# Blosc/c-blosc

Measured on NVIDIA H100. Metric: compress+decompress GB/s, higher is better.
Workload: dtype u8

## Files before the change

c-blosc_b200/csrc/dev_lz4.cuh:

```cuda
#pragma once
#include "dev_common.cuh"

#define LZ4_MFLIMIT 12
#define LZ4_LASTLITERALS 5
#define LZ4_TABLE_BYTES 16384
#define LZ4_TAB17_BYTES (8192 + 512)
#define LZ4_TAB17_MINLEN 65547
#define LZ4_TAB17_MAXLEN 131072

template <bool U16>
DEV u32 lz4_hash_at(const u8* __restrict__ s, int pos) {
  if (U16) return (ld_u32(s + pos) * 2654435761u) >> (32 - 13);
  const u64 seq = (u64)ld_u32(s + pos) | ((u64)s[pos + 4] << 32);
  return (u32)(((seq << 24) * 889523592379ull) >> (64 - 12));
}

#define LZ4_SCALAR_PROBES 4

DEV long long lz4_probe_offset(int it, int accel) {
  if (it == 0) return 0;
  const long long m = it - 1;
  const long long c = m >> 6;
  return 1 + m * accel + 32 * c * (c - 1) + c * (m - 64 * c);
}

struct StreamBase {
  const u8* s;
  const u32* s32;
  int sal;
  const uint4* s128;
  int sal16;
};
DEV StreamBase make_stream_base(const u8* s) {
  StreamBase b;
  b.s = s;
  b.s32 = (const u32*)((uintptr_t)s & ~(uintptr_t)3);
  b.sal = (int)((uintptr_t)s & 3u);
  b.s128 = (const uint4*)((uintptr_t)s & ~(uintptr_t)15);
  b.sal16 = (int)((uintptr_t)s & 15u);
  return b;
}
DEV void ldp_win12(const StreamBase& sb, int p, u32& b0, u32& b1, u32& b2) {
#ifdef SIMT_EMU
  memcpy(&b0, sb.s + p, 4); memcpy(&b1, sb.s + p + 4, 4); memcpy(&b2, sb.s + p + 8, 4);
#else
  const int q = p + sb.sal;
  const u32* w = sb.s32 + (q >> 2);
  const u32 sh = (u32)(q & 3) * 8u;
  const u32 w0 = __ldg(w), w1 = __ldg(w + 1), w2 = __ldg(w + 2), w3 = __ldg(w + 3);
  b0 = __funnelshift_r(w0, w1, sh); b1 = __funnelshift_r(w1, w2, sh); b2 = __funnelshift_r(w2, w3, sh);
#endif
}
DEV void ldp_raw12(const StreamBase& sb, int p, u32& r0, u32& r1, u32& r2, u32& r3) {
#ifdef SIMT_EMU
  memcpy(&r0, sb.s + p, 4); memcpy(&r1, sb.s + p + 4, 4); memcpy(&r2, sb.s + p + 8, 4); r3 = 0;
#else
  const u32* w = sb.s32 + ((p + sb.sal) >> 2);
  r0 = __ldg(w); r1 = __ldg(w + 1); r2 = __ldg(w + 2); r3 = __ldg(w + 3);
#endif
}
DEV void ldp_take12(const StreamBase& sb, int p, u32 r0, u32 r1, u32 r2, u32 r3, u32& b0, u32& b1, u32& b2) {
#ifdef SIMT_EMU
  (void)sb; (void)p; (void)r3; b0 = r0; b1 = r1; b2 = r2;
#else
  const u32 sh = (u32)((p + sb.sal) & 3) * 8u;
  b0 = __funnelshift_r(r0, r1, sh); b1 = __funnelshift_r(r1, r2, sh); b2 = __funnelshift_r(r2, r3, sh);
#endif
}
DEV void ldp_win8(const StreamBase& sb, int p, u32& b0, u32& b1) {
#ifdef SIMT_EMU
  memcpy(&b0, sb.s + p, 4); memcpy(&b1, sb.s + p + 4, 4);
#else
  const int q = p + sb.sal;
  const u32* w = sb.s32 + (q >> 2);
  const u32 sh = (u32)(q & 3) * 8u;
  const u32 w0 = __ldg(w), w1 = __ldg(w + 1), w2 = __ldg(w + 2);
  b0 = __funnelshift_r(w0, w1, sh); b1 = __funnelshift_r(w1, w2, sh);
#endif
}

DEV void ldp_raw20(const StreamBase& sb, int p, u32 (&r)[5]) {
#ifdef SIMT_EMU
  memcpy(&r[0], sb.s + p, 16); r[4] = sb.s[p + 16];
#else
  const u32* w = sb.s32 + ((p + sb.sal) >> 2);
  r[0] = __ldg(w); r[1] = __ldg(w + 1); r[2] = __ldg(w + 2); r[3] = __ldg(w + 3); r[4] = __ldg(w + 4);
#endif
}
DEV void ldp_take17(const StreamBase& sb, int p, const u32 (&r)[5], u32& a0, u32& a1, u32& a2, u32& a3, u32& a4b) {
#ifdef SIMT_EMU
  (void)sb; (void)p; a0 = r[0]; a1 = r[1]; a2 = r[2]; a3 = r[3]; a4b = r[4] & 0xffu;
#else
  const u32 sh = (u32)((p + sb.sal) & 3) * 8u;
  a0 = __funnelshift_r(r[0], r[1], sh); a1 = __funnelshift_r(r[1], r[2], sh);
  a2 = __funnelshift_r(r[2], r[3], sh); a3 = __funnelshift_r(r[3], r[4], sh);
  a4b = (r[4] >> sh) & 0xffu;
#endif
}
DEV void ldp_gather17(const StreamBase& sb, int p, u32& c0, u32& c1, u32& c2, u32& c3, u32& c4b) {
#ifdef SIMT_EMU
  memcpy(&c0, sb.s + p, 4); memcpy(&c1, sb.s + p + 4, 4); memcpy(&c2, sb.s + p + 8, 4); memcpy(&c3, sb.s + p + 12, 4);
  c4b = sb.s[p + 16];
#else
  const int q = p + sb.sal16;
  const uint4* w = sb.s128 + (q >> 4);
  const uint4 v0 = __ldg(w), v1 = __ldg(w + 1);
  const bool k1 = (q & 4) != 0, k2 = (q & 8) != 0;
  const u32 sh = (u32)(q & 3) * 8u;
  const u32 t0 = k1 ? v0.y : v0.x, t1 = k1 ? v0.z : v0.y, t2 = k1 ? v0.w : v0.z, t3 = k1 ? v1.x : v0.w;
  const u32 t4 = k1 ? v1.y : v1.x, t5 = k1 ? v1.z : v1.y, t6 = k1 ? v1.w : v1.z;
  const u32 u0 = k2 ? t2 : t0, u1 = k2 ? t3 : t1, u2 = k2 ? t4 : t2, u3 = k2 ? t5 : t3, u4 = k2 ? t6 : t4;
  c0 = __funnelshift_r(u0, u1, sh); c1 = __funnelshift_r(u1, u2, sh);
  c2 = __funnelshift_r(u2, u3, sh); c3 = __funnelshift_r(u3, u4, sh);
  c4b = (u4 >> sh) & 0xffu;
#endif
}

DEV void lz4d_prefetch(const u8* base, int p, int end) {
#ifndef SIMT_EMU
  if (p < end) asm volatile("prefetch.global.L1 [%0];" :: "l"(base + p));
#else
  (void)base; (void)p; (void)end;
#endif
}

DEV u32 ldp_win4(const StreamBase& sb, int p) {
#ifdef SIMT_EMU
  u32 b0; memcpy(&b0, sb.s + p, 4); return b0;
#else
  const int q = p + sb.sal;
  const u32* w = sb.s32 + (q >> 2);
  return __funnelshift_r(__ldg(w), __ldg(w + 1), (u32)(q & 3) * 8u);
#endif
}

template <bool U16>
DEV u32 lz4_hash_seq(u32 lo, u32 b4) {
  if (U16) return (lo * 2654435761u) >> (32 - 13);
  const u64 seq = (u64)lo | ((u64)(b4 & 0xffu) << 32);
  return (u32)(((seq << 24) * 889523592379ull) >> (64 - 12));
}

DEV int lz4_count_tail(const StreamBase& sb, const u8* __restrict__ s, int p, int q, int limit, int n) {
  if (p + 136 <= n) {
    const int lane = lane_id();
    const u32 x = ldp_win4(sb, p + 4 * lane) ^ ldp_win4(sb, q + 4 * lane);
    const unsigned full = __ballot_sync(FULLMASK, x == 0u);
    if (full != FULLMASK) {
      const int fl = __ffs((int)~full) - 1;
      return fl * 4 + eq_bytes32(__shfl_sync(FULLMASK, x, fl));
    }
    return 128 + warp_count_match(s, p + 128, q + 128, limit);
  }
  return warp_count_match(s, p, q, limit);
}

#ifdef SIMT_EMU
static long long g_dbg_lz4t_sessions = 0, g_dbg_lz4t_seqs = 0, g_dbg_lz4t_stale = 0, g_dbg_lz4t_x[6];
#define LZ4T_DBG(x) do { if (lane_id() == 0) (x)++; } while (0)
#else
#define LZ4T_DBG(x) do {} while (0)
#endif
#ifndef LZ4T_TILES
#define LZ4T_TILES 12
#endif
#ifndef LZ4T_AHEAD
#define LZ4T_AHEAD 8
#endif
#ifndef LZ4T_NAP
#define LZ4T_NAP 128
#endif
#define LZ4T_RING (32 * LZ4T_TILES)
#define LZ4T_BAR_IDLE(i) (1 + (i))
#define LZ4T_BAR_GO(i) (4 + (i))
#define LZ4T_QUIT 1
#define LZ4T_STOP 0x7fffffff
#define LZ4T_END 0xffffffffu
#define LZ4T_LONG 13
static_assert(LZ4T_TILES % 3 == 0 && LZ4T_AHEAD >= 1 && LZ4T_AHEAD < LZ4T_TILES && LZ4T_RING > 15 + 255 + 4, "team ring layout");
#define LZ4T_PREFETCH 512

enum {
  LZ4C_TOTAL,
  LZ4C_START,
  LZ4C_SESSION,
  LZ4C_FULLWAIT,
  LZ4C_REPROBE,
  LZ4C_SEARCH,
  LZ4C_SESSIONS, LZ4C_SEQS, LZ4C_CHAIN_SEQS,
  LZ4C_PREP_BUSY,
  LZ4C_PREP_OWN,
  LZ4C_PREP_GATHER,
  LZ4C_PREP_TILES,
  LZ4C_SMID, LZ4C_SUBP,
  LZ4C_STALE,
  LZ4C_N = 16
};
#ifdef B2_LZ4_CYCLES
#define LZ4C_MAXSTREAMS 16384
__device__ unsigned long long g_lz4_cycles[LZ4C_MAXSTREAMS][LZ4C_N];
#define LZ4C_T(t) const long long t = clock64()
#define LZ4C_TW(t) const long long t = TEAM ? clock64() : 0ll
#define LZ4C_ADD(k, v) do { if (lane_id() == 0) atomicAdd(&tm->cyc[k], (unsigned long long)(v)); } while (0)
#define LZ4C_SPAN(k, t) LZ4C_ADD(k, clock64() - (t))
#else
#define LZ4C_T(t) do {} while (0)
#define LZ4C_TW(t) do {} while (0)
#define LZ4C_ADD(k, v) do {} while (0)
#define LZ4C_SPAN(k, t) do {} while (0)
#endif

struct Lz4Team {
  uint2 vd[LZ4T_RING];
  int rdy[LZ4T_TILES];
  const u8* s;
  int n;
  int u16;
  int wt;
  int gen;
  int cmd;
  int sub[4];
  int slot;
#ifdef B2_LZ4_CYCLES
  unsigned long long cyc[LZ4C_N];
#endif
};
#define LZ4T_SMEM_BYTES ((int)sizeof(Lz4Team))

DEV int lz4t_ld_i32(const int* p) { return *(const volatile int*)p; }
DEV void lz4t_st_i32(int* p, int v) { *(volatile int*)p = v; }

template <bool U16>
DEV void lz4_team_prepare_tile(Lz4Team* tm, const void* tabmem, const u8* s, int n, int tile) {
  const int lane = lane_id();
  const int w0 = 32 * tile, p = w0 + lane;
  const int e = (tile % LZ4T_TILES) * 32 + lane;
  if (w0 + 31 + 24 > n) { tm->vd[e] = make_uint2(0u, LZ4T_END); return; }
  const StreamBase sb = make_stream_base(s);
  u32 r[5], a0, a1, a2, a3, a4, c0, c1, c2, c3, c4;
  LZ4C_T(c_t0);
  ldp_raw20(sb, p, r);
  ldp_take17(sb, p, r, a0, a1, a2, a3, a4);
  const u32 h = lz4_hash_seq<U16>(a0, a1);
  const int snap = U16 ? (int)((const volatile u16*)tabmem)[h] : (int)((const volatile u32*)tabmem)[h];
  u32 vx = h << 8, sn = LZ4T_END;
  if ((unsigned)snap < (unsigned)p) {
    LZ4C_T(c_t1);
    LZ4C_ADD(LZ4C_PREP_OWN, c_t1 - c_t0);
    ldp_gather17(sb, snap, c0, c1, c2, c3, c4);
    const u32 x1 = a1 ^ c1, x2 = a2 ^ c2, x3 = a3 ^ c3;
    u32 m;
    if (x1) m = (u32)(__ffs((int)x1) - 1) >> 3;
    else if (x2) m = 4u + ((u32)(__ffs((int)x2) - 1) >> 3);
    else if (x3) m = 8u + ((u32)(__ffs((int)x3) - 1) >> 3);
    else m = a4 != c4 ? 12u : (u32)LZ4T_LONG;
    const bool hit = (U16 || snap + 65535 >= p) && c0 == a0;
    vx |= (hit ? 1u : 0u) | (m << 2);
    sn = (u32)snap;
    LZ4C_SPAN(LZ4C_PREP_GATHER, c_t1);
  }
  tm->vd[e] = make_uint2(vx, sn);
}

DEV void lz4_team_preparer(Lz4Team* tm, const void* tabmem, int i) {
  for (;;) {
    bar_sync(LZ4T_BAR_GO(i), 64);
    if (lz4t_ld_i32(&tm->cmd) == LZ4T_QUIT) return;
    const u8* s = *(const u8* const volatile*)&tm->s;
    const int n = lz4t_ld_i32(&tm->n), u16 = lz4t_ld_i32(&tm->u16);
    for (int tile = i;; tile += 3) {
      int w;
      for (;;) {
        w = __shfl_sync(FULLMASK, lz4t_ld_i32(&tm->wt), 0);
        if (w == LZ4T_STOP) break;
        if (tile < w) tile = w + (i + 3 - w % 3) % 3;
        if (tile <= w + LZ4T_AHEAD) break;
        __nanosleep(LZ4T_NAP);
      }
      if (w == LZ4T_STOP) break;
      LZ4C_T(c_go);
      lz4d_prefetch(s, 32 * tile + LZ4T_PREFETCH + lane_id(), n);
      if (u16) lz4_team_prepare_tile<true>(tm, tabmem, s, n, tile);
      else lz4_team_prepare_tile<false>(tm, tabmem, s, n, tile);
      __syncwarp();
      if (lane_id() == 0) { __threadfence_block(); lz4t_st_i32(&tm->rdy[tile % LZ4T_TILES], tile + 1); }
      LZ4C_SPAN(LZ4C_PREP_BUSY, c_go);
      LZ4C_ADD(LZ4C_PREP_TILES, 1);
    }
    __syncwarp();
    bar_arrive(LZ4T_BAR_IDLE(i), 64);
  }
}

DEV void lz4t_reach(Lz4Team* tm, int ip, int& wt, int& vt) {
  const int lo = (ip - 2) >> 5, hi = ip >> 5;
  if (lo > wt + LZ4T_AHEAD) LZ4T_DBG(g_dbg_lz4t_x[2]);
  if (lo != wt) { wt = lo; lz4t_st_i32(&tm->wt, lo); }
  for (int t = vt + 1 > lo ? vt + 1 : lo; t <= hi; t++) {
    const int* r = &tm->rdy[t % LZ4T_TILES];
    if (lz4t_ld_i32(r) != t + 1) {
      LZ4T_DBG(g_dbg_lz4t_x[5]);
      do { __syncwarp(); } while (__any_sync(FULLMASK, lz4t_ld_i32(r) != t + 1));
    }
  }
  if (hi > vt) vt = hi;
}

template <bool U16, bool PACK, bool TEAM>
DEV int lz4_encode_stream(const u8* __restrict__ s, const int n, u8* __restrict__ d, const int cap,
                          const int accel, void* tabmem, int* need_out, Lz4Team* tm) {
  const int lane = lane_id();
  const StreamBase sb = make_stream_base(s);
  u16* tab16 = (u16*)tabmem;
  u32* tab32 = (u32*)tabmem;
  u32* tabhi = (u32*)((u8*)tabmem + 8192);
#define LZ4_TGET(h) (U16 ? (int)tab16[h] : PACK ? ((int)tab16[h] | (int)(((tabhi[(h) >> 5] >> ((h) & 31u)) & 1u) << 16)) : (int)tab32[h])
#define LZ4_TPUT(h, v) do { if (U16) tab16[h] = (u16)(v); else if (PACK) { tab16[h] = (u16)(v); const u32 m_ = 1u << ((h) & 31u); \
                            if ((v) & 0x10000) atomicOr(&tabhi[(h) >> 5], m_); else atomicAnd(&tabhi[(h) >> 5], ~m_); } \
                            else tab32[h] = (u32)(v); } while (0)

  for (int i = lane; i < (PACK ? LZ4_TAB17_BYTES : LZ4_TABLE_BYTES) / 4; i += 32) tab32[i] = 0;
  __syncwarp();

  const bool limited = (long long)cap < (long long)n + n / 255 + 16;
  const int olimit = cap;
  const int mfl1 = n - LZ4_MFLIMIT + 1;
  const int matchlimit = n - LZ4_LASTLITERALS;
  int ip = 1, anchor = 0, op = 0;
  int need = 0;
#define LZ4_LIMIT(v) do { const int v_ = (v); if (v_ > need) need = v_; if (limited && v_ > olimit) return 0; } while (0)

  int w0 = -(1 << 30);
  u32 wq0 = 0, wq1 = 0, wq2 = 0, wh = 0;
  int pb = -(1 << 30);
  u32 pq0 = 0, pq1 = 0, pq2 = 0, pq3 = 0;
  int nrec = 0, recop = 0;
  u32 rec = 0;
  int twt = 0, tvt = -1;
#define LZ4_FLUSH_CHECKED() do { if (nrec) { LZ4_LIMIT(op + (1 + LZ4_LASTLITERALS)); } LZ4_FLUSH(); } while (0)
#define LZ4_FLUSH() do { if (lane < nrec) { d[recop] = (u8)rec; d[recop + 1] = (u8)(rec >> 8); d[recop + 2] = (u8)(rec >> 16); \
                                             if ((rec & 15u) == 15u) d[recop + 3] = (u8)(rec >> 24); } nrec = 0; } while (0)

  if (n >= LZ4_MFLIMIT + 1) {
    bool post = false;
    for (;;) {
      int match = 0, lit = 0, back = 0;
      u32 ipn = 0, cn = 0;
      bool have_next = false, hit = false, imm = false, have_mc = false;
      int mc_carry = 0;

      bool scalar_post = post;
      if (TEAM && post && ip + 64 <= n) {
        scalar_post = false;
        bool finished = false;
        if (nrec >= 24) LZ4_FLUSH_CHECKED();
        LZ4T_DBG(g_dbg_lz4t_sessions);
        LZ4C_T(c_s0);
        LZ4C_ADD(LZ4C_SESSIONS, 1);
        if ((ip - 2) >> 5 <= twt + LZ4T_AHEAD) LZ4T_DBG(g_dbg_lz4t_x[3]);
        lz4t_reach(tm, ip, twt, tvt);
        __syncwarp();
        LZ4C_SPAN(LZ4C_START, c_s0);
        LZ4C_T(c_s1);
        const smem_addr_t vda = smem_addr(tm->vd);
        u32 e = (u32)ip % (u32)LZ4T_RING;
        for (;;) {
          u32 pk, snap;
          smem_ld_u32x2(vda, e << 3, pk, snap);
          const u32 h2 = smem_ld_u32(vda, (e >= 2u ? e - 2u : e - 2u + LZ4T_RING) << 3) >> 8;
          const u32 h = pk >> 8;
          LZ4_TPUT(h2, ip - 2);
          const int cand = LZ4_TGET(h);
          __syncwarp();
          if (cand != (int)snap) {
            LZ4T_DBG(g_dbg_lz4t_stale); LZ4C_ADD(LZ4C_STALE, 1);
            scalar_post = true; break;
          }
          LZ4_TPUT(h, ip);
          if (!(pk & 1u)) { LZ4T_DBG(g_dbg_lz4t_x[4]); ip++; break; }
          const int off = ip - (int)snap;
          int mc = (int)((pk >> 2) & 15u);
          if (mc == LZ4T_LONG) {
            LZ4T_DBG(g_dbg_lz4t_x[0]);
            mc = LZ4T_LONG + lz4_count_tail(sb, s, ip + 4 + LZ4T_LONG, ip - off + 4 + LZ4T_LONG, matchlimit, n);
            if (mc >= 15 + 255) {
              hit = true; imm = true; match = ip - off;
              have_mc = true; mc_carry = mc;
              LZ4T_DBG(g_dbg_lz4t_x[1]);
              break;
            }
          }
          const bool ext = mc >= 15;
          LZ4T_DBG(g_dbg_lz4t_seqs);
          LZ4C_ADD(LZ4C_CHAIN_SEQS, 1);
          if (lane == nrec) { rec = (ext ? 15u | ((u32)(mc - 15) << 24) : (u32)mc) | ((u32)off << 8); recop = op; }
          nrec++;
          op += ext ? 4 : 3;
          ip += mc + 4;
          e += (u32)(mc + 4);
          if (e >= (u32)LZ4T_RING) e -= (u32)LZ4T_RING;
          anchor = ip;
          if (ip + 64 > n) {
            if (ip >= mfl1) finished = true;
            else scalar_post = true;
            break;
          }
          if ((ip >> 5) > tvt) {
            LZ4C_T(c_w);
            lz4t_reach(tm, ip, twt, tvt);
            LZ4C_SPAN(LZ4C_FULLWAIT, c_w);
            if (nrec >= 24) LZ4_FLUSH_CHECKED();
          }
        }
        LZ4C_SPAN(LZ4C_SESSION, c_s1);
        if (finished) break;
      }
      if (!TEAM && post && ip + 64 <= n) {
        scalar_post = false;
        bool room = true;
        for (;;) {
          if (ip - 2 < w0 || ip > w0 + 31) {
            if (nrec >= 24) LZ4_FLUSH_CHECKED();
            if (ip - 2 >= pb && ip <= pb + 31) { w0 = pb; ldp_take12(sb, w0 + lane, pq0, pq1, pq2, pq3, wq0, wq1, wq2); }
            else { w0 = ip - 2; ldp_win12(sb, w0 + lane, wq0, wq1, wq2); }
            wh = lz4_hash_seq<U16>(wq0, wq1);
            pb = w0 + 30;
            if (pb + 31 + 16 <= n) ldp_raw12(sb, pb + lane, pq0, pq1, pq2, pq3);
            else pb = -(1 << 30);
            lz4d_prefetch(s, w0 + 192, lane == 0 ? n : 0);
          }
          const int li = ip - w0;
          const u32 h2 = __shfl_sync(FULLMASK, wh, li - 2);
          const u32 h = __shfl_sync(FULLMASK, wh, li);
          const u32 seq = __shfl_sync(FULLMASK, wq0, li);
          const u32 n4 = __shfl_sync(FULLMASK, wq1, li);
          const u32 n8 = __shfl_sync(FULLMASK, wq2, li);
          if (lane == 0) LZ4_TPUT(h2, ip - 2);
          __syncwarp();
          const int cand = LZ4_TGET(h);
          __syncwarp();
          if (lane == 0) LZ4_TPUT(h, ip);
          u32 c0, c1, c2;
          ldp_win12(sb, cand, c0, c1, c2);
          if (!((U16 || cand + 65535 >= ip) && c0 == seq)) { ip++; break; }
          int mc;
          const u32 x1 = n4 ^ c1, x2 = n8 ^ c2;
          if (x1 | x2) {
            const u32 xx = x1 ? x1 : x2;
            mc = ((__ffs((int)xx) - 1) >> 3) + (x1 ? 0 : 4);
          } else {
            u32 p3, p4, q3, q4;
            ldp_win8(sb, ip + 12, p3, p4);
            ldp_win8(sb, cand + 12, q3, q4);
            const u32 x3 = p3 ^ q3, x4 = p4 ^ q4;
            if (x3) mc = 8 + eq_bytes32(x3);
            else if (x4) mc = 12 + eq_bytes32(x4);
            else mc = 16 + lz4_count_tail(sb, s, ip + 20, cand + 20, matchlimit, n);
          }
          if (mc >= 15 + 255) {
            hit = true; imm = true; match = cand;
            have_mc = true; mc_carry = mc;
            break;
          }
          const bool ext = mc >= 15;
          const int off = ip - cand;
          if (lane == nrec) { rec = (ext ? 15u | ((u32)(mc - 15) << 24) : (u32)mc) | ((u32)off << 8); recop = op; }
          nrec++;
          op += ext ? 4 : 3;
          ip += mc + 4;
          anchor = ip;
          if (ip + 64 > n) { room = false; break; }
        }
        if (!room) {
          if (ip >= mfl1) break;
          continue;
        }
      }
      if (scalar_post) {
        LZ4C_TW(c_r);
        u32 b0, b1, b2 = 0;
        const bool wide = ip + 14 <= n;
        if (wide) ldp_win12(sb, ip - 2, b0, b1, b2);
        else { b0 = ld_u32(s + ip - 2); b1 = ld_u32(s + ip + 2); }
        const u32 seq = __funnelshift_r(b0, b1, 16);
        const u32 h2 = lz4_hash_seq<U16>(b0, b1);
        const u32 h = lz4_hash_seq<U16>(seq, b1 >> 16);
        if (lane == 0) LZ4_TPUT(h2, ip - 2);
        __syncwarp();
        const int cand = LZ4_TGET(h);
        __syncwarp();
        if (lane == 0) LZ4_TPUT(h, ip);
        if (U16 || cand + 65535 >= ip) {
          u32 c0, c1;
          ldp_win8(sb, cand, c0, c1);
          if (c0 == seq) {
            hit = true; imm = true; match = cand;
            ipn = __funnelshift_r(b1, b2, 16); cn = c1; have_next = wide;
          }
        }
        if (!hit) ip++;
        if (TEAM) LZ4C_SPAN(LZ4C_REPROBE, c_r);
      }

      if (!hit) {
        LZ4C_TW(c_f);
        bool ended = false;
        for (int it = 0; it < LZ4_SCALAR_PROBES; it++) {
          const int pos = ip + (it ? 1 + (it - 1) * accel : 0);
          if (ip + 1 + it * accel > mfl1) { ended = true; break; }
          u32 b0, b1 = 0, b2 = 0;
          const bool wide = pos + 16 <= n;
          if (wide) ldp_win12(sb, pos, b0, b1, b2);
          else { b0 = ld_u32(s + pos); b1 = (u32)s[pos + 4]; }
          const u32 h = lz4_hash_seq<U16>(b0, b1);
          __syncwarp();
          const int cand = LZ4_TGET(h);
          __syncwarp();
          if (lane == 0) LZ4_TPUT(h, pos);
          if (U16 || cand + 65535 >= pos) {
            u32 c0, c1;
            ldp_win8(sb, cand, c0, c1);
            if (c0 == b0) {
              hit = true; ip = pos; match = cand;
              ipn = b1; cn = c1; have_next = wide;
              break;
            }
          }
        }
        if (!hit && !ended) {
          __syncwarp();
          for (int base_it = LZ4_SCALAR_PROBES;; base_it += 32) {
            const int itl = base_it + lane;
            const bool valid = ip + lz4_probe_offset(itl + 1, accel) <= mfl1;
            const int pos = valid ? ip + (int)lz4_probe_offset(itl, accel) : 0;
            u32 h = 0x80000000u | (u32)lane, seq = 0;
            if (valid) { seq = ld_u32(s + pos); h = lz4_hash_at<U16>(s, pos); }
            const unsigned vmask = __ballot_sync(FULLMASK, valid);
            const unsigned peers = __match_any_sync(FULLMASK, h);
            const unsigned lower = peers & ((1u << lane) - 1u);
            int cand = 0;
            bool lhit = false;
            if (valid) {
              cand = lower ? ip + (int)lz4_probe_offset(base_it + (31 - __clz((int)lower)), accel) : LZ4_TGET(h);
              if (U16 || cand + 65535 >= pos) lhit = ld_u32(s + cand) == seq;
            }
            const unsigned found = __ballot_sync(FULLMASK, lhit);
            const int nvalid = __popc(vmask);
            const int f = found ? __ffs((int)found) - 1 : 32;
            const int last = f < nvalid - 1 ? f : nvalid - 1;
            __syncwarp();
            if (valid && lane <= last) {
              const unsigned le = last >= 31 ? FULLMASK : ((1u << (last + 1)) - 1u);
              if ((((peers & le) >> lane) >> 1) == 0) LZ4_TPUT(h, pos);
            }
            __syncwarp();
            if (found) {
              ip = __shfl_sync(FULLMASK, pos, f);
              match = __shfl_sync(FULLMASK, cand, f);
              hit = true;
              break;
            }
            if (nvalid < 32) break;
          }
        }
        if (!hit) { if (TEAM) LZ4C_SPAN(LZ4C_SEARCH, c_f); break; }

        if (ip > anchor && match > 0 && s[ip - 1] == s[match - 1]) {
          for (;;) {
            const int a = ip - 1 - back - lane, b = match - 1 - back - lane;
            const bool ok = a >= anchor && b >= 0 && s[a] == s[b];
            const unsigned m = __ballot_sync(FULLMASK, ok);
            const int step = m == FULLMASK ? 32 : __ffs((int)~m) - 1;
            back += step;
            if (step < 32) break;
          }
        }
        lit = ip - back - anchor;
        if (TEAM) LZ4C_SPAN(LZ4C_SEARCH, c_f);
      }

      int mc;
      if (have_mc) mc = mc_carry;
      else {
        const int room = matchlimit - (ip + 4);
        if (have_next) {
          const u32 x = ipn ^ cn;
          if (x) mc = eq_bytes32(x);
          else if (room > 20) {
            u32 p0, p1, p2, q0, q1, q2;
            ldp_win12(sb, ip + 8, p0, p1, p2);
            ldp_win12(sb, match + 8, q0, q1, q2);
            const u32 x0 = p0 ^ q0, x1 = p1 ^ q1, x2 = p2 ^ q2;
            if (x0) mc = 4 + eq_bytes32(x0);
            else if (x1) mc = 8 + eq_bytes32(x1);
            else if (x2) mc = 12 + eq_bytes32(x2);
            else mc = 16 + lz4_count_tail(sb, s, ip + 20, match + 20, matchlimit, n);
          } else mc = 4 + (room > 4 ? warp_count_match(s, ip + 8, match + 8, matchlimit) : 0);
          if (mc > room) mc = room;
        } else mc = warp_count_match(s, ip + 4, match + 4, matchlimit);
      }
      const int off = ip - match;
      ip += mc + 4;
      mc += back;

      if (TEAM) LZ4C_ADD(LZ4C_SEQS, 1);
      LZ4_FLUSH_CHECKED();
      const int token = op++;
      if (!imm) LZ4_LIMIT(op + lit + (2 + 1 + LZ4_LASTLITERALS) + lit / 255);
      if (lit < 15 && mc < 15) {
        LZ4_LIMIT(op + lit + 2 + (1 + LZ4_LASTLITERALS));
        u32 v;
        if (lane == 0) v = ((u32)lit << 4) | (u32)mc;
        else if (lane <= lit) v = s[anchor + lane - 1];
        else v = lane == lit + 1 ? (u32)off : (u32)off >> 8;
        if (lane <= lit + 2) d[token + lane] = (u8)v;
        op += lit + 2;
      } else {
        u32 tokval;
        if (lit >= 15) {
          const int len = lit - 15, nff = len / 255;
          tokval = 15u << 4;
          warp_fill_bytes(d + op, nff, 255);
          if (lane == 0) d[op + nff] = (u8)(len - nff * 255);
          op += nff + 1;
        } else tokval = (u32)lit << 4;
        warp_copy_bytes(d + op, s + anchor, lit);
        op += lit;
        if (lane == 0) { d[op] = (u8)off; d[op + 1] = (u8)(off >> 8); }
        op += 2;
        LZ4_LIMIT(op + (1 + LZ4_LASTLITERALS) + (mc + 240) / 255);
        if (mc >= 15) {
          tokval += 15;
          const int rest = mc - 15, nff = rest / 255;
          warp_fill_bytes(d + op, nff, 255);
          if (lane == 0) d[op + nff] = (u8)(rest - nff * 255);
          op += nff + 1;
        } else tokval += (u32)mc;
        if (lane == 0) d[token] = (u8)tokval;
      }

      anchor = ip;
      if (ip >= mfl1) break;
      post = true;
    }
  }

  LZ4_FLUSH_CHECKED();
  const int lastRun = n - anchor;
  LZ4_LIMIT(op + lastRun + 1 + (lastRun + 255 - 15) / 255);
  if (lastRun >= 15) {
    const int acc = lastRun - 15, nff = acc / 255;
    if (lane == 0) d[op] = (u8)(15u << 4);
    op++;
    warp_fill_bytes(d + op, nff, 255);
    if (lane == 0) d[op + nff] = (u8)(acc - nff * 255);
    op += nff + 1;
  } else {
    if (lane == 0) d[op] = (u8)(lastRun << 4);
    op++;
  }
  warp_copy_bytes(d + op, s + anchor, lastRun);
  op += lastRun;
  *need_out = need;
  return op;
#undef LZ4_FLUSH_CHECKED
#undef LZ4_FLUSH
#undef LZ4_LIMIT
#undef LZ4_TGET
#undef LZ4_TPUT
}

DEV void lz4t_begin(Lz4Team* tm, const u8* s, int n, bool u16) {
  const int lane = lane_id();
  for (int i = lane; i < LZ4T_TILES; i += 32) tm->rdy[i] = 0;
  if (lane == 0) { tm->s = s; tm->n = n; tm->u16 = u16 ? 1 : 0; tm->wt = 0; tm->gen = tm->gen + 1; }
  __syncwarp();
  __threadfence_block();
  bar_arrive(LZ4T_BAR_GO(0), 64); bar_arrive(LZ4T_BAR_GO(1), 64); bar_arrive(LZ4T_BAR_GO(2), 64);
}
DEV void lz4t_end(Lz4Team* tm) {
  if (lane_id() == 0) lz4t_st_i32(&tm->wt, LZ4T_STOP);
  __syncwarp();
  bar_sync(LZ4T_BAR_IDLE(0), 64); bar_sync(LZ4T_BAR_IDLE(1), 64); bar_sync(LZ4T_BAR_IDLE(2), 64);
}

template <bool U16, bool PACK = false, bool TEAM = false>
DEV int lz4_encode_warp(const u8* __restrict__ s, const int n, u8* __restrict__ d, const int cap,
                        const int accel, void* tabmem, int* need_out, Lz4Team* tm = nullptr) {
  if (TEAM) lz4t_begin(tm, s, n, U16);
  const int c = lz4_encode_stream<U16, PACK, TEAM>(s, n, d, cap, accel, tabmem, need_out, tm);
  if (TEAM) lz4t_end(tm);
  return c;
}

enum {
  LZ4D_H_DENSE_SHIFT = 0,
  LZ4D_H_DENSE_LONGCAP = 9,
  LZ4D_H_DENSE_BAD,
  LZ4D_H_DENSE_BAD0,
  LZ4D_H_DENSE_FEW,
  LZ4D_H_DENSE_RING, LZ4D_H_DENSE_GLOBAL,
  LZ4D_H_LONE_RING, LZ4D_H_LONE_GLOBAL, LZ4D_H_LONE_PERIOD,
  LZ4D_H_BATCH_FAST, LZ4D_H_BATCH_WALK,
  LZ4D_H_BATCH_RING, LZ4D_H_BATCH_GLOBAL,
  LZ4D_H_SINGLE_RING, LZ4D_H_SINGLE_GLOBAL,
  LZ4D_H_GEN_LITBUMP,
  LZ4D_H_GEN_OFF0, LZ4D_H_GEN_RING, LZ4D_H_GEN_GLOBAL, LZ4D_H_GEN_LONG, LZ4D_H_GEN_LAST,
  LZ4D_NHIT
};
#ifdef SIMT_EMU
static long long g_dbg_lz4d_batch_seqs = 0, g_dbg_lz4d_fast_seqs = 0, g_dbg_lz4d_general_seqs = 0, g_dbg_lz4d_dense_seqs = 0;
#define LZ4D_DBG(x) do { if (lane == 0) (x)++; } while (0)
#define LZ4D_DBGN(x, n) do { if (lane == 0) (x) += (n); } while (0)
static int g_lz4d_fail_line = 0;
#define LZ4D_FAIL (g_lz4d_fail_line = g_lz4d_fail_line ? g_lz4d_fail_line : __LINE__, -1)
static long long g_lz4d_hit[LZ4D_NHIT];
#define LZ4D_HIT(id) do { if (lane == 0) g_lz4d_hit[id]++; } while (0)
#define LZ4D_HITL(id, c) do { if (c) g_lz4d_hit[id]++; } while (0)
#else
#define LZ4D_DBG(x) do {} while (0)
#define LZ4D_DBGN(x, n) do {} while (0)
#define LZ4D_FAIL (-1)
#define LZ4D_HIT(id) do {} while (0)
#define LZ4D_HITL(id, c) do {} while (0)
#endif
#define LZ4D_RING 16384
#define LZ4D_RMASK (LZ4D_RING - 1)
#define LZ4D_BATCH_OUT 320
#define LZ4D_DENSE_LONG 8
#define LZ4D_DENSE_OUT 2624
#define LZ4D_DENSE_MIN 4
#define LZ4D_SCRATCH 256
#define LZ4D_SMEM (LZ4D_RING + LZ4D_SCRATCH)

enum { LZ4D_ZERO = 0, LZ4D_FROM_RING = 1, LZ4D_FROM_GLOBAL = 2, LZ4D_LONG = 3 };
#define LZ4D_TBL_START 22

DEV void lz4d_copy_dense(u8* out, smem_addr_t ring, int dst, int off, int ml, int kind, bool from_ring, int cnt,
                         unsigned longm) {
  const int lane = lane_id();
  const int match = dst - off;
  {
    const int mls = (lane < cnt && kind == 1) ? ml : 0;
    const int mlmax = __ballot_sync(FULLMASK, mls > 16) ? 18 : (__ballot_sync(FULLMASK, mls > 8) ? 16 : 8);
    u8* o = out + dst;
#pragma unroll 1
    for (int k = 0; k < mlmax; k += 4) {
      if (k < mls) {
        u32 v;
        if (from_ring) {
          const u32 m = (u32)(match + k);
          v = __funnelshift_r(smem_ld_u32(ring, m & (LZ4D_RMASK & ~3u)), smem_ld_u32(ring, (m + 4u) & (LZ4D_RMASK & ~3u)), (m & 3u) * 8u);
        } else v = ld_u32(out + match + k);
        const int nb = mls - k;
        const u32 r = (u32)(dst + k);
        o[k] = (u8)v; smem_st_u8(ring, r & LZ4D_RMASK, v);
        if (nb > 1) { o[k + 1] = (u8)(v >> 8); smem_st_u8(ring, (r + 1u) & LZ4D_RMASK, v >> 8); }
        if (nb > 2) { o[k + 2] = (u8)(v >> 16); smem_st_u8(ring, (r + 2u) & LZ4D_RMASK, v >> 16); }
        if (nb > 3) { o[k + 3] = (u8)(v >> 24); smem_st_u8(ring, (r + 3u) & LZ4D_RMASK, v >> 24); }
      }
    }
  }
  for (unsigned tm = longm; tm; tm &= tm - 1u) {
    const int t = __ffs((int)tm) - 1;
    const int td = __shfl_sync(FULLMASK, dst, t), tmt = __shfl_sync(FULLMASK, match, t), tl = __shfl_sync(FULLMASK, ml, t);
    const bool tring = __shfl_sync(FULLMASK, (int)from_ring, t) != 0;
    for (int k = lane; k < tl; k += 32) {
      const u32 v = tring ? smem_ld_u8(ring, (u32)(tmt + k) & LZ4D_RMASK) : (u32)out[tmt + k];
      out[td + k] = (u8)v;
      smem_st_u8(ring, (u32)(td + k) & LZ4D_RMASK, v);
    }
  }
}

DEV void lz4d_copy_lone(u8* out, smem_addr_t ring, int op, int len, int off, bool from_ring) {
  const int match = op - off;
  for (int k = lane_id(); k < len; k += 32) {
    const int src = match + (off >= len ? k : k % off);
    const u32 v = from_ring ? smem_ld_u8(ring, (u32)src & LZ4D_RMASK) : (u32)out[src];
    out[op + k] = (u8)v;
    smem_st_u8(ring, (u32)(op + k) & LZ4D_RMASK, v);
  }
}

DEV void lz4d_batch_table(u32* tbl, int my_rank, int my_opre, int lit, int off) {
  const int lane = lane_id();
  if (lane < 10) tbl[LZ4D_TBL_START + lane] = 0;
  __syncwarp();
  if (my_rank >= 0) {
    tbl[2 * my_rank] = (u32)my_opre | ((u32)lit << 9) | ((u32)lane << 13);
    tbl[2 * my_rank + 1] = (u32)off;
    atomicOr(&tbl[LZ4D_TBL_START + (my_opre >> 5)], 1u << (my_opre & 31));
  }
}

DEV void lz4d_copy_batch(const u8* in, u8* out, smem_addr_t ring, int ip, int op, int total, int ring_lo, const u32* tbl) {
  const int lane = lane_id();
  int kbase = 0;
  for (int r = 0; r * 32 < total; r++) {
    const u32 w = tbl[LZ4D_TBL_START + r];
    const int y = r * 32 + lane;
    if (y < total) {
      const int k = kbase + __popc(w & ((2u << lane) - 1u)) - 1;
      const u32 e0 = tbl[2 * k], offk = tbl[2 * k + 1];
      const int opre = (int)(e0 & 511u), litk = (int)((e0 >> 9) & 15u), lanek = (int)(e0 >> 13);
      const int j = y - opre;
      u32 v;
      if (j < litk) v = in[ip + lanek + 1 + j];
      else {
        const int src = op + opre + litk - (int)offk + (j - litk);
        const int m0 = op + opre + litk - (int)offk;
        if ((int)offk <= LZ4D_RING - LZ4D_BATCH_OUT - 64 && m0 >= ring_lo) v = smem_ld_u8(ring, (u32)src & LZ4D_RMASK);
        else v = out[src];
      }
      out[op + y] = (u8)v;
      smem_st_u8(ring, (u32)(op + y) & LZ4D_RMASK, v);
    }
    kbase += __popc(w);
  }
}

DEV void lz4d_copy_single(const u8* in, u8* out, smem_addr_t ring, int ip, int op, int lit, int total, int off,
                          bool use_ring) {
  const int lane = lane_id();
  const int match = op + lit - off;
  if (lane < total) {
    u32 v;
    if (lane < lit) v = in[ip + 1 + lane];
    else if (use_ring) v = smem_ld_u8(ring, (u32)(match + lane - lit) & LZ4D_RMASK);
    else v = out[match + lane - lit];
    out[op + lane] = (u8)v;
    smem_st_u8(ring, (u32)(op + lane) & LZ4D_RMASK, v);
  }
}

DEV void lz4d_copy_general(const u8* in, u8* out, smem_addr_t ring, int lsrc, int op, int len, int mlen, int off, int how) {
  const int lane = lane_id();
  for (int k = lane; k < len; k += 32) {
    const u32 v = in[lsrc + k];
    out[op + k] = (u8)v;
    smem_st_u8(ring, (u32)(op + k) & LZ4D_RMASK, v);
  }
  if (mlen == 0) return;
  op += len;
  const int match = op - off;
  __syncwarp();
  if (how == LZ4D_ZERO) {
    for (int k = lane; k < mlen; k += 32) out[op + k] = 0;
  } else if (how != LZ4D_LONG) {
    const bool from_ring = how == LZ4D_FROM_RING;
    for (int k0 = 0; k0 < mlen; k0 += 32) {
      const int k = k0 + lane;
      if (k < mlen) {
        const int src = match + (off >= mlen ? k : k % off);
        const u32 v = from_ring ? smem_ld_u8(ring, (u32)src & LZ4D_RMASK) : (u32)out[src];
        out[op + k] = (u8)v;
        smem_st_u8(ring, (u32)(op + k) & LZ4D_RMASK, v);
      }
    }
  } else warp_copy_match(out, op, match, mlen);
}

struct Lz4dWarpCopies {
  const u8* in;
  u8* out;
  u8* ring_ptr;
  smem_addr_t ring;
  DEV Lz4dWarpCopies(u8* out_, u8* ring_ptr_) : in(nullptr), out(out_), ring_ptr(ring_ptr_), ring(smem_addr(ring_ptr_)) {}
  DEV void start(const u8* in_) { in = in_; }
  DEV void dense(int dst, int off, int ml, int kind, bool from_ring, int cnt, unsigned longm) {
    lz4d_copy_dense(out, ring, dst, off, ml, kind, from_ring, cnt, longm);
    __syncwarp();
  }
  DEV void lone(int op, int len, int off, bool from_ring) { lz4d_copy_lone(out, ring, op, len, off, from_ring); __syncwarp(); }
  DEV u32* batch_table() { return (u32*)(ring_ptr + LZ4D_RING); }
  DEV void batch(int ip, int op, int total, int ring_lo) {
    __syncwarp();
    lz4d_copy_batch(in, out, ring, ip, op, total, ring_lo, batch_table());
    __syncwarp();
  }
  DEV void single(int ip, int op, int lit, int total, int off, bool use_ring) {
    lz4d_copy_single(in, out, ring, ip, op, lit, total, off, use_ring);
    __syncwarp();
  }
  DEV void literals(int lsrc, int op, int len) { lz4d_copy_general(in, out, ring, lsrc, op, len, 0, 0, LZ4D_ZERO); }
  DEV void match(int op, int mlen, int off, int how) {
    lz4d_copy_general(in, out, ring, 0, op, 0, mlen, off, how);
    __syncwarp();
  }
  DEV void finish() {}
};

template <class Copies>
DEV int lz4d_walk(const u8* __restrict__ in, const int csize, const int cap, Copies& cp) {
  const int iend = csize, oend = cap;
  const int lane = lane_id();
  const StreamBase ib = make_stream_base(in);
  int ip = 0, op = 0, result = 0;
  int ring_lo = 0;
  if (cap == 0) return (csize == 1 && in[0] == 0) ? 0 : LZ4D_FAIL;
  if (csize == 0) return LZ4D_FAIL;
  cp.start(in);
  int dense_skip = 0, dense_back = 0;
  for (;;) {
    if (dense_skip > 0) dense_skip--;
    else if (ip + 112 <= iend && op + LZ4D_DENSE_OUT <= oend - LZ4_MFLIMIT) {
      u32 b0, b1, b2;
      ldp_win12(ib, ip + 3 * lane, b0, b1, b2);
      lz4d_prefetch(in, ip + 256 + 128 * lane, lane < 2 ? iend : 0);
      int kind = 0, ml = 0, off = 0, c = 0, sft = 0;
      u32 w = b0;
      for (;;) {
        const u32 tok = w & 0xffu;
        const unsigned okm = __ballot_sync(FULLMASK, lane >= c && (tok >> 4) == 0u && (tok & 15u) != 15u);
        const unsigned stop = ~okm & ~((1u << c) - 1u);
        const int e = stop ? __ffs((int)stop) - 1 : 32;
        if (lane >= c && lane < e) { kind = 1; ml = (int)(tok & 15u) + 4; off = (int)((w >> 8) & 0xffffu); }
        c = e;
        if (e >= 32 || sft == LZ4D_DENSE_LONG) break;
        const u32 tw = __shfl_sync(FULLMASK, w, e);
        if ((tw & 0xffu) != 0x0fu || (tw >> 24) == 255u) break;
        if (lane == e) { kind = 2; ml = 19 + (int)(tw >> 24); off = (int)((tw >> 8) & 0xffffu); }
        c = e + 1; sft++;
        if (c >= 32) break;
        w = sft < 4 ? __funnelshift_r(b0, b1, 8u * (u32)sft) : (sft == 4 ? b1 : (sft < 8 ? __funnelshift_r(b1, b2, 8u * (u32)(sft - 4)) : b2));
      }
      int cnt = c;
      int incl = ml;
#pragma unroll
      for (int d = 1; d < 32; d <<= 1) {
        const int t = __shfl_up_sync(FULLMASK, incl, d);
        if (lane >= d) incl += t;
      }
      const int dst = op + incl - ml, match = dst - off;
      const unsigned bad = __ballot_sync(FULLMASK, lane < cnt && (off < incl + 8 || match < 0));
      if (bad) cnt = __ffs((int)bad) - 1;
      if (bad) LZ4D_HIT(cnt == 0 ? LZ4D_H_DENSE_BAD0 : LZ4D_H_DENSE_BAD);
      const unsigned longm = __ballot_sync(FULLMASK, lane < cnt && kind == 2);
      if (cnt >= LZ4D_DENSE_MIN || longm) {
        const int total = __shfl_sync(FULLMASK, incl, cnt - 1);
        const bool from_ring = off <= LZ4D_RING - LZ4D_DENSE_OUT - 64 && match >= ring_lo;
        LZ4D_HIT(LZ4D_H_DENSE_SHIFT + sft);
        if (sft == LZ4D_DENSE_LONG && c < 32) LZ4D_HIT(LZ4D_H_DENSE_LONGCAP);
        LZ4D_HITL(from_ring ? LZ4D_H_DENSE_RING : LZ4D_H_DENSE_GLOBAL, lane < cnt);
        cp.dense(dst, off, ml, kind, from_ring, cnt, longm);
        ip += 3 * cnt + __popc(longm); op += total;
        LZ4D_DBGN(g_dbg_lz4d_dense_seqs, cnt);
        dense_back = 0;
        continue;
      }
      {
        const u32 tw = __shfl_sync(FULLMASK, b0, 0);
        const int tlen = 19 + (int)(tw >> 24), toff = (int)((tw >> 8) & 0xffffu), tmatch = op - toff;
        if ((tw & 0xffu) == 0x0fu && (tw >> 24) != 255u && toff != 0 && tmatch >= 0 && op + tlen <= oend - LZ4_MFLIMIT) {
          const bool tring = toff <= LZ4D_RING - 512 && tmatch >= ring_lo;
          LZ4D_HIT(tring ? LZ4D_H_LONE_RING : LZ4D_H_LONE_GLOBAL);
          if (toff < tlen) LZ4D_HIT(LZ4D_H_LONE_PERIOD);
          cp.lone(op, tlen, toff, tring);
          ip += 4; op += tlen;
          LZ4D_DBG(g_dbg_lz4d_dense_seqs);
          dense_back = 0;
          continue;
        }
      }
      if (cnt > 0) LZ4D_HIT(LZ4D_H_DENSE_FEW);
      dense_back = dense_back < 8 ? dense_back + 1 : 8;
      dense_skip = dense_back;
    }
    if (ip + 49 <= iend && op + LZ4D_BATCH_OUT <= oend - LZ4_MFLIMIT) {
      u32 b0, b1, b2;
      ldp_win12(ib, ip + lane, b0, b1, b2);
      const u32 token = b0 & 0xffu;
      const int lit = (int)(token >> 4), mln = (int)(token & 15u);
      const int ob = 1 + lit;
      const u32 ow = ob < 4 ? __funnelshift_r(b0, b1, 8u * ob) : (ob < 8 ? __funnelshift_r(b1, b2, 8u * (ob - 4)) : b2 >> (8u * ((ob - 8) & 3)));
      const int off = (int)(ow & 0xffffu);
      const int L = 3 + lit, O = lit + mln + 4;
      const bool good = lit <= 9 && mln != 15 && off >= LZ4D_BATCH_OUT;
      int nseq = 0, consumed = 0, total = 0, my_rank = -1, my_opre = 0;
      const unsigned g3 = __ballot_sync(FULLMASK, good && lit == 0);
      if ((g3 & 0x49249249u) == 0x49249249u) {
        const bool real = (lane % 3) == 0;
        const int v = real ? O : 0;
        int incl = v;
#pragma unroll
        for (int d = 1; d < 32; d <<= 1) {
          const int t = __shfl_up_sync(FULLMASK, incl, d);
          if (lane >= d) incl += t;
        }
        if (real) { my_rank = lane / 3; my_opre = incl - v; }
        nseq = 11; consumed = 33;
        total = __shfl_sync(FULLMASK, incl, 31);
      } else {
        const u32 packed = (good ? 1u : 0u) | ((u32)L << 1) | ((u32)O << 5);
        int cur = 0;
        while (cur < 32) {
          const u32 pk = __shfl_sync(FULLMASK, packed, cur);
          if (!(pk & 1u)) break;
          if (lane == cur) { my_rank = nseq; my_opre = total; }
          total += (int)((pk >> 5) & 31u);
          cur += (int)((pk >> 1) & 15u);
          nseq++;
        }
        consumed = cur;
      }
      if (nseq > 0) {
        const int match = op + my_opre + lit - off;
        if (__ballot_sync(FULLMASK, my_rank >= 0 && match < 0)) { result = LZ4D_FAIL; break; }
        LZ4D_HIT((g3 & 0x49249249u) == 0x49249249u ? LZ4D_H_BATCH_FAST : LZ4D_H_BATCH_WALK);
        LZ4D_HITL(off <= LZ4D_RING - LZ4D_BATCH_OUT - 64 && match >= ring_lo ? LZ4D_H_BATCH_RING : LZ4D_H_BATCH_GLOBAL, my_rank >= 0);
        lz4d_batch_table(cp.batch_table(), my_rank, my_opre, lit, off);
        cp.batch(ip, op, total, ring_lo);
        ip += consumed; op += total;
        LZ4D_DBGN(g_dbg_lz4d_batch_seqs, nseq);
        continue;
      }
    }
    if (ip + 20 <= iend) {
      u32 b0, b1, b2;
      ldp_win12(ib, ip, b0, b1, b2);
      const u32 token = b0 & 0xffu;
      const int lit = (int)(token >> 4), mln = (int)(token & 15u);
      if (lit <= 9 && mln != 15) {
        const int ml = mln + 4, total = lit + ml;
        const int ob = 1 + lit;
        const u32 ow = ob < 4 ? __funnelshift_r(b0, b1, 8u * ob) : (ob < 8 ? __funnelshift_r(b1, b2, 8u * (ob - 4)) : b2 >> (8u * (ob - 8)));
        const int off = (int)(ow & 0xffffu);
        const int match = op + lit - off;
        if (off >= total && op + total <= oend - LZ4_MFLIMIT) {
          if (match < 0) { result = LZ4D_FAIL; break; }
          const bool use_ring = off <= LZ4D_RING - 64 && match >= ring_lo;
          LZ4D_HIT(use_ring ? LZ4D_H_SINGLE_RING : LZ4D_H_SINGLE_GLOBAL);
          cp.single(ip, op, lit, total, off, use_ring);
          ip += 3 + lit; op += total;
          LZ4D_DBG(g_dbg_lz4d_fast_seqs);
          continue;
        }
      }
    }
    LZ4D_DBG(g_dbg_lz4d_general_seqs);
    const u32 token = in[ip++];
    int len = (int)(token >> 4);
    if (len == 15) {
      u32 sb;
      if (ip >= iend - 15) { result = LZ4D_FAIL; break; }
      do {
        sb = in[ip++];
        len += (int)sb;
        if (ip > iend - 15) { result = LZ4D_FAIL; break; }
        if (len > oend) { result = LZ4D_FAIL; break; }
      } while (sb == 255);
      if (result < 0) break;
    }
    int cpy = op + len;
    const bool last = cpy > oend - LZ4_MFLIMIT || ip + len > iend - (2 + 1 + LZ4_LASTLITERALS);
    if (last && (ip + len != iend || cpy > oend)) { result = LZ4D_FAIL; break; }
    cp.literals(ip, op, len);
    if (len > LZ4D_RING - 64) { ring_lo = cpy - (LZ4D_RING - 64) > ring_lo ? cpy - (LZ4D_RING - 64) : ring_lo; LZ4D_HIT(LZ4D_H_GEN_LITBUMP); }
    if (last) { LZ4D_HIT(LZ4D_H_GEN_LAST); result = cpy; break; }
    ip += len; op = cpy;
    const int off = (int)in[ip] | ((int)in[ip + 1] << 8);
    ip += 2;
    const int match = op - off;
    int mlen = (int)(token & 15u);
    if (mlen == 15) {
      u32 sb;
      do {
        sb = in[ip++];
        mlen += (int)sb;
        if (ip > iend - LZ4_LASTLITERALS + 1) { result = LZ4D_FAIL; break; }
        if (mlen > oend) { result = LZ4D_FAIL; break; }
      } while (sb == 255);
      if (result < 0) break;
    }
    mlen += 4;
    if (match < 0) { result = LZ4D_FAIL; break; }
    cpy = op + mlen;
    if (cpy > oend - LZ4_LASTLITERALS) { result = LZ4D_FAIL; break; }
    int how = LZ4D_ZERO;
    if (off == 0) {
      ring_lo = cpy;
      LZ4D_HIT(LZ4D_H_GEN_OFF0);
    } else if (mlen <= 2048) {
      how = off <= LZ4D_RING - 2048 - 64 && match >= ring_lo ? LZ4D_FROM_RING : LZ4D_FROM_GLOBAL;
      LZ4D_HIT(how == LZ4D_FROM_RING ? LZ4D_H_GEN_RING : LZ4D_H_GEN_GLOBAL);
    } else {
      how = LZ4D_LONG;
      ring_lo = cpy;
      LZ4D_HIT(LZ4D_H_GEN_LONG);
    }
    cp.match(op, mlen, off, how);
    op = cpy;
  }
  cp.finish();
  __syncwarp();
  return result;
}

DEV int lz4_decode_warp(const u8* __restrict__ in, const int csize, u8* out, const int cap, u8* ring_ptr) {
  Lz4dWarpCopies cp(out, ring_ptr);
  return lz4d_walk(in, csize, cap, cp);
}
```

Measured before the change: 111.0.

## Precompute backward-match extent in team preparers and probe via prepared tiles

The preparer warps now also compute how many bytes a hit extends backwards (up to 7), packing it into the tile descriptor, and the hash is moved to a higher bit shift. When the team session reaches a miss, the encoder now runs the next few accelerated probes from the prepared ring instead of dropping to the scalar warp search. It can fold short literal runs straight into a chained sequence. This cuts per-match hash gathers and backward scans on the critical encoder warp. The cost is extra preparer work and more branching, with a fallback to the old catch-up when the backward cap is reached.

```diff
diff --git a/c-blosc_b200/csrc/dev_lz4.cuh b/c-blosc_b200/csrc/dev_lz4.cuh
--- a/c-blosc_b200/csrc/dev_lz4.cuh
+++ b/c-blosc_b200/csrc/dev_lz4.cuh
@@ -155,8 +155,31 @@
   return warp_count_match(s, p, q, limit);
 }
 
+DEV int lz4_catch_up(const u8* __restrict__ s, int ip, int match, int anchor, int back) {
+  const int lane = lane_id();
+  for (;;) {
+    const int a = ip - 1 - back - lane, b = match - 1 - back - lane;
+    const bool ok = a >= anchor && b >= 0 && s[a] == s[b];
+    const unsigned m = __ballot_sync(FULLMASK, ok);
+    const int step = m == FULLMASK ? 32 : __ffs((int)~m) - 1;
+    back += step;
+    if (step < 32) return back;
+  }
+}
+
 #ifdef SIMT_EMU
 static long long g_dbg_lz4t_sessions = 0, g_dbg_lz4t_seqs = 0, g_dbg_lz4t_stale = 0, g_dbg_lz4t_x[6];
+enum {
+  LZ4T_S_HIT0,
+  LZ4T_S_STALE = 4,
+  LZ4T_S_MISS4,
+  LZ4T_S_LIT,
+  LZ4T_S_CAPPED,
+  LZ4T_S_LONG,
+  LZ4T_S_HUGE,
+  LZ4T_S_N
+};
+static long long g_dbg_lz4t_s[LZ4T_S_N];
 #define LZ4T_DBG(x) do { if (lane_id() == 0) (x)++; } while (0)
 #else
 #define LZ4T_DBG(x) do {} while (0)
@@ -177,6 +200,8 @@
 #define LZ4T_STOP 0x7fffffff
 #define LZ4T_END 0xffffffffu
 #define LZ4T_LONG 13
+#define LZ4T_HSHIFT 19
+#define LZ4T_BACKCAP 7
 static_assert(LZ4T_TILES % 3 == 0 && LZ4T_AHEAD >= 1 && LZ4T_AHEAD < LZ4T_TILES && LZ4T_RING > 15 + 255 + 4, "team ring layout");
 #define LZ4T_PREFETCH 512
 
@@ -243,7 +268,7 @@
   ldp_take17(sb, p, r, a0, a1, a2, a3, a4);
   const u32 h = lz4_hash_seq<U16>(a0, a1);
   const int snap = U16 ? (int)((const volatile u16*)tabmem)[h] : (int)((const volatile u32*)tabmem)[h];
-  u32 vx = h << 8, sn = LZ4T_END;
+  u32 vx = h << LZ4T_HSHIFT, sn = LZ4T_END;
   if ((unsigned)snap < (unsigned)p) {
     LZ4C_T(c_t1);
     LZ4C_ADD(LZ4C_PREP_OWN, c_t1 - c_t0);
@@ -255,7 +280,19 @@
     else if (x3) m = 8u + ((u32)(__ffs((int)x3) - 1) >> 3);
     else m = a4 != c4 ? 12u : (u32)LZ4T_LONG;
     const bool hit = (U16 || snap + 65535 >= p) && c0 == a0;
-    vx |= (hit ? 1u : 0u) | (m << 2);
+    u32 bk = 0;
+    if (hit) {
+      if (snap >= 8) {
+        u32 p0, p1, q0, q1;
+        ldp_win8(sb, p - 8, p0, p1);
+        ldp_win8(sb, snap - 8, q0, q1);
+        const u32 y1 = p1 ^ q1, z0 = (u32)__clz((int)(p0 ^ q0)) >> 3;
+        bk = y1 ? (u32)__clz((int)y1) >> 3 : 4u + (z0 < 3u ? z0 : 3u);
+      } else {
+        while (bk < (u32)snap && s[p - 1 - (int)bk] == s[snap - 1 - (int)bk]) bk++;
+      }
+    }
+    vx |= (hit ? 1u : 0u) | (m << 2) | (bk << 8);
     sn = (u32)snap;
     LZ4C_SPAN(LZ4C_PREP_GATHER, c_t1);
   }
@@ -304,6 +341,58 @@
     }
   }
   if (hi > vt) vt = hi;
+}
+
+template <bool U16>
+DEV bool lz4t_search(Lz4Team* tm, smem_addr_t vda, void* tabmem, const StreamBase& sb, int n, int anchor, int accel,
+                     int& twt, int& tvt, u32& pk, u32& snap, int& ip, bool& hit, int& match, int& back, int& lit,
+                     bool& have_mc, int& mc_carry) {
+  u16* tab16 = (u16*)tabmem;
+  u32* tab32 = (u32*)tabmem;
+  const int mfl1 = n - LZ4_MFLIMIT + 1;
+  ip = anchor + 1;
+  int it = 0, pos = ip;
+  for (;; it++) {
+    if (it == LZ4_SCALAR_PROBES) { LZ4T_DBG(g_dbg_lz4t_s[LZ4T_S_MISS4]); lit = it; return false; }
+    pos = ip + (it ? 1 + (it - 1) * accel : 0);
+    if (ip + 1 + it * accel > mfl1) { lit = it; return false; }
+    if ((pos >> 5) > tvt) lz4t_reach(tm, pos, twt, tvt);
+    u32 qk, qs;
+    smem_ld_u32x2(vda, ((u32)pos % (u32)LZ4T_RING) << 3, qk, qs);
+    const u32 h = qk >> LZ4T_HSHIFT;
+    const int cand = U16 ? (int)tab16[h] : (int)tab32[h];
+    __syncwarp();
+    if (cand != (int)qs) { LZ4T_DBG(g_dbg_lz4t_s[LZ4T_S_STALE]); lit = it; return false; }
+    if (U16) tab16[h] = (u16)pos; else tab32[h] = (u32)pos;
+    if (qk & 1u) { pk = qk; snap = qs; break; }
+  }
+  LZ4T_DBG(g_dbg_lz4t_s[LZ4T_S_HIT0 + it]);
+  const int vb = (int)((pk >> 8) & 7u), dist = pos - anchor;
+  const int bq = vb < dist ? vb : dist;
+  int m = (int)((pk >> 2) & 15u);
+  if (m == LZ4T_LONG) {
+    LZ4T_DBG(g_dbg_lz4t_s[LZ4T_S_LONG]);
+    m = LZ4T_LONG + lz4_count_tail(sb, sb.s, pos + 4 + LZ4T_LONG, (int)snap + 4 + LZ4T_LONG, n - LZ4_LASTLITERALS, n);
+  }
+  if (bq == dist && bq + m < 15 + 255) {
+    const int mc = bq + m;
+    snap -= (u32)bq;
+    pk = 1u | ((u32)(mc < LZ4T_LONG ? mc : LZ4T_LONG) << 2);
+    ip = anchor;
+    LZ4C_ADD(LZ4C_SEQS, 1);
+    LZ4C_ADD(LZ4C_CHAIN_SEQS, ~0ull);
+    return true;
+  }
+  hit = true; ip = pos; match = (int)snap;
+  have_mc = true; mc_carry = m;
+  back = bq;
+  if (vb == LZ4T_BACKCAP && dist > LZ4T_BACKCAP) {
+    LZ4T_DBG(g_dbg_lz4t_s[LZ4T_S_CAPPED]);
+    back = lz4_catch_up(sb.s, pos, (int)snap, anchor, LZ4T_BACKCAP);
+  } else if (bq != dist) LZ4T_DBG(g_dbg_lz4t_s[LZ4T_S_LIT]);
+  else LZ4T_DBG(g_dbg_lz4t_s[LZ4T_S_HUGE]);
+  lit = pos - back - anchor;
+  return false;
 }
 
 template <bool U16, bool PACK, bool TEAM>
@@ -367,8 +456,8 @@
         for (;;) {
           u32 pk, snap;
           smem_ld_u32x2(vda, e << 3, pk, snap);
-          const u32 h2 = smem_ld_u32(vda, (e >= 2u ? e - 2u : e - 2u + LZ4T_RING) << 3) >> 8;
-          const u32 h = pk >> 8;
+          const u32 h2 = smem_ld_u32(vda, (e >= 2u ? e - 2u : e - 2u + LZ4T_RING) << 3) >> LZ4T_HSHIFT;
+          const u32 h = pk >> LZ4T_HSHIFT;
           LZ4_TPUT(h2, ip - 2);
           const int cand = LZ4_TGET(h);
           __syncwarp();
@@ -377,7 +466,14 @@
             scalar_post = true; break;
           }
           LZ4_TPUT(h, ip);
-          if (!(pk & 1u)) { LZ4T_DBG(g_dbg_lz4t_x[4]); ip++; break; }
+          if (!(pk & 1u)) {
+            LZ4T_DBG(g_dbg_lz4t_x[4]);
+            if constexpr (TEAM) {
+              if (!lz4t_search<U16>(tm, vda, tabmem, sb, n, anchor, accel, twt, tvt, pk, snap, ip, hit, match, back, lit, have_mc, mc_carry))
+                break;
+              if (nrec >= 24) LZ4_FLUSH_CHECKED();
+            } else { ip++; break; }
+          }
           const int off = ip - (int)snap;
           int mc = (int)((pk >> 2) & 15u);
           if (mc == LZ4T_LONG) {
@@ -505,7 +601,7 @@
       if (!hit) {
         LZ4C_TW(c_f);
         bool ended = false;
-        for (int it = 0; it < LZ4_SCALAR_PROBES; it++) {
+        for (int it = TEAM ? lit : 0; it < LZ4_SCALAR_PROBES; it++) {
           const int pos = ip + (it ? 1 + (it - 1) * accel : 0);
           if (ip + 1 + it * accel > mfl1) { ended = true; break; }
           u32 b0, b1 = 0, b2 = 0;
@@ -565,16 +661,7 @@
         }
         if (!hit) { if (TEAM) LZ4C_SPAN(LZ4C_SEARCH, c_f); break; }
 
-        if (ip > anchor && match > 0 && s[ip - 1] == s[match - 1]) {
-          for (;;) {
-            const int a = ip - 1 - back - lane, b = match - 1 - back - lane;
-            const bool ok = a >= anchor && b >= 0 && s[a] == s[b];
-            const unsigned m = __ballot_sync(FULLMASK, ok);
-            const int step = m == FULLMASK ? 32 : __ffs((int)~m) - 1;
-            back += step;
-            if (step < 32) break;
-          }
-        }
+        if (ip > anchor && match > 0 && s[ip - 1] == s[match - 1]) back = lz4_catch_up(s, ip, match, anchor, 0);
         lit = ip - back - anchor;
         if (TEAM) LZ4C_SPAN(LZ4C_SEARCH, c_f);
       }
@@ -679,6 +766,7 @@
   bar_arrive(LZ4T_BAR_GO(0), 64); bar_arrive(LZ4T_BAR_GO(1), 64); bar_arrive(LZ4T_BAR_GO(2), 64);
 }
 DEV void lz4t_end(Lz4Team* tm) {
+  __syncwarp();
   if (lane_id() == 0) lz4t_st_i32(&tm->wt, LZ4T_STOP);
   __syncwarp();
   bar_sync(LZ4T_BAR_IDLE(0), 64); bar_sync(LZ4T_BAR_IDLE(1), 64); bar_sync(LZ4T_BAR_IDLE(2), 64);
```

After: 121.9, median of 6. 1.1x the previous value.
